# ruizhecao96/CMGAN

Hardware: NVIDIA H100
Metric: utterances/sec (2 s @16 kHz) generator fwd+bwd (higher is better)
Workload: dtype tf32

## Files before the change

### cmgan_b200/csrc/attention_mma.cu

```cuda
#include <type_traits>

#include "common.cuh"
#include "../../include/cmgan_b200.h"
#include "tc_ptx.cuh"

namespace {
using cmgan_tc::cp_async16;
using cmgan_tc::cp_async_commit;
using cmgan_tc::cp_async_wait;
using cmgan_tc::smem_u32;

constexpr int D = 16, H = 4, CQ = 64, LDQ = 192;
constexpr int QB = 64;
constexpr int KT = 64;
constexpr int LDS_ = 20;
constexpr int EW = QB + KT - 1;
constexpr int RW = 80;
constexpr int LDR = 84;
constexpr int MAXPOS = 512;
constexpr float SCALE_LOG2E = 0.25f * 1.4426950408889634f;

__device__ __forceinline__ float tf32r(float x) {
    uint32_t r;
    asm("cvt.rna.tf32.f32 %0, %1;" : "=r"(r) : "f"(x));
    return __uint_as_float(r);
}
__device__ __forceinline__ float tf32q(float x) { return __uint_as_float(__float_as_uint(x) + 0x1000u); }
__device__ __forceinline__ float ex2(float x) {
    float y;
    asm("ex2.approx.ftz.f32 %0, %1;" : "=f"(y) : "f"(x));
    return y;
}
__device__ __forceinline__ void mma_tf32(float c[4], const float a[4], float b0, float b1) {
    asm volatile("mma.sync.aligned.m16n8k8.row.col.f32.tf32.tf32.f32 {%0, %1, %2, %3}, {%4, %5, %6, %7}, {%8, %9}, {%0, %1, %2, %3};"
                 : "+f"(c[0]), "+f"(c[1]), "+f"(c[2]), "+f"(c[3])
                 : "r"(__float_as_uint(a[0])), "r"(__float_as_uint(a[1])), "r"(__float_as_uint(a[2])), "r"(__float_as_uint(a[3])),
                   "r"(__float_as_uint(b0)), "r"(__float_as_uint(b1)));
}
__device__ __forceinline__ int clampi(int v, int lo, int hi) { return v < lo ? lo : (v > hi ? hi : v); }

constexpr int EROWS = EW + 1;
constexpr int TILE_FLOATS = 2 * KT * LDS_ + EROWS * LDS_;
__device__ __forceinline__ void stage_tile_async(float* buf, const float* __restrict__ a_src, int a_ld, const float* __restrict__ b_src, int b_ld,
                                                 long base, long tok_stride, int first, int L, const float* __restrict__ E, int rfirst, int tid) {
    const uint32_t sa = smem_u32(buf), sb = sa + KT * LDS_ * 4, se = sb + KT * LDS_ * 4;
    for (int idx = tid; idx < KT * 4; idx += 128) {
        const int r = idx >> 2, q4 = idx & 3;
        const bool ok = first + r < L;
        const long row = base + (long)(ok ? first + r : 0) * tok_stride;
        cp_async16(sa + (r * LDS_ + q4 * 4) * 4, a_src + row * a_ld + q4 * 4, ok ? 16u : 0u);
        cp_async16(sb + (r * LDS_ + q4 * 4) * 4, b_src + row * b_ld + q4 * 4, ok ? 16u : 0u);
    }
    for (int idx = tid; idx < EROWS * 4; idx += 128) {
        const int w = idx >> 2, q4 = idx & 3;
        const int e = clampi(rfirst + w, -MAXPOS, MAXPOS) + MAXPOS;
        cp_async16(se + (w * LDS_ + q4 * 4) * 4, E + e * D + q4 * 4, 16u);
    }
}

template <int NBUF, bool RAGGED>
__global__ void __launch_bounds__(128) attn_fwd_mma_kernel(const float* __restrict__ qkv, SeqGeom g, const float* __restrict__ E,
                                                           float* __restrict__ ctx, float* __restrict__ lse, const int* __restrict__ tlen,
                                                           int axis) {
    extern __shared__ __align__(16) float smem_fwd[];
    float* Rs0 = smem_fwd + NBUF * TILE_FLOATS;
    const int s = blockIdx.x / H, h = blockIdx.x % H;
    const int i0 = blockIdx.y * QB;
    const int tid = threadIdx.x, warp = tid >> 5, lane = tid & 31, gq = lane >> 2, t = lane & 3;
    const int L = RAGGED ? ragged_seq_len(g, s, tlen, axis) : g.L;
    if (RAGGED && i0 >= L) return;
    const long base = seq_base(g, s);
    const int iw = i0 + warp * 16;
    const bool warp_active = iw < L;

    float qa[2][4];
#pragma unroll
    for (int ks = 0; ks < 2; ++ks)
#pragma unroll
        for (int r = 0; r < 4; ++r) {
            const int row = iw + gq + (r & 1) * 8, col = t + (r >> 1) * 4 + ks * 8;
            float v = 0.f;
            if (row < L) v = __ldg(qkv + (base + (long)row * g.tok_stride) * LDQ + h * D + col) * SCALE_LOG2E;
            qa[ks][r] = tf32r(v);
        }
    float o[2][4];
#pragma unroll
    for (int nd = 0; nd < 2; ++nd)
#pragma unroll
        for (int r = 0; r < 4; ++r) o[nd][r] = 0.f;
    float mrun[2] = {-INFINITY, -INFINITY}, lrun[2] = {0.f, 0.f};

    const float* ksrc = qkv + h * D + CQ;
    const float* vsrc = qkv + h * D + 2 * CQ;
    if (NBUF == 2) {
        stage_tile_async(smem_fwd, ksrc, LDQ, vsrc, LDQ, base, g.tok_stride, 0, L, E, i0 - (KT - 1), tid);
        cp_async_commit();
    }
    for (int j0 = 0, it = 0; j0 < L; j0 += KT, ++it) {
        const int nk = min(KT, L - j0);
        const float* Ks = smem_fwd + (NBUF == 2 ? (it & 1) : 0) * TILE_FLOATS;
        const float* Vs = Ks + KT * LDS_;
        const float* Es = Vs + KT * LDS_;
        __syncthreads();
        if (NBUF == 2) {
            if (j0 + KT < L)
                stage_tile_async(smem_fwd + ((it + 1) & 1) * TILE_FLOATS, ksrc, LDQ, vsrc, LDQ, base, g.tok_stride, j0 + KT, L, E,
                                 i0 - (j0 + KT) - (KT - 1), tid);
            cp_async_commit();
            cp_async_wait<1>();
        } else {
            stage_tile_async(smem_fwd, ksrc, LDQ, vsrc, LDQ, base, g.tok_stride, j0, L, E, i0 - j0 - (KT - 1), tid);
            cp_async_commit();
            cp_async_wait<0>();
        }
        __syncthreads();
        if (!warp_active) continue;
        auto tile_body = [&](auto full_tag) {
        constexpr bool FULL = decltype(full_tag)::value;
        const int ntv = (nk + 7) >> 3;
        const int rt0 = (KT - nk) >> 3;

        float sc[8][4];
#pragma unroll
        for (int nt = 0; nt < 8; ++nt) {
            sc[nt][0] = sc[nt][1] = sc[nt][2] = sc[nt][3] = 0.f;
            if (!FULL && nt >= ntv) continue;
#pragma unroll
            for (int ks = 0; ks < 2; ++ks) {
                const float* kp = Ks + (nt * 8 + gq) * LDS_ + t + ks * 8;
                mma_tf32(sc[nt], qa[ks], kp[0], kp[4]);
            }
        }
        float* R = Rs0 + warp * 16 * LDR;
#pragma unroll
        for (int nt = 0; nt < RW / 8; ++nt) {
            if (!FULL && nt < rt0) continue;
            float rc[4] = {0.f, 0.f, 0.f, 0.f};
#pragma unroll
            for (int ks = 0; ks < 2; ++ks) {
                const float* ep = Es + (warp * 16 + nt * 8 + gq) * LDS_ + t + ks * 8;
                mma_tf32(rc, qa[ks], ep[0], ep[4]);
            }
            *reinterpret_cast<float2*>(R + gq * LDR + nt * 8 + 2 * t) = make_float2(rc[0], rc[1]);
            *reinterpret_cast<float2*>(R + (gq + 8) * LDR + nt * 8 + 2 * t) = make_float2(rc[2], rc[3]);
        }
        __syncwarp();
        float tmax[2] = {-INFINITY, -INFINITY};
#pragma unroll
        for (int nt = 0; nt < 8; ++nt) {
            if (!FULL && nt >= ntv) { sc[nt][0] = sc[nt][1] = sc[nt][2] = sc[nt][3] = -INFINITY; continue; }
#pragma unroll
            for (int r = 0; r < 4; ++r) {
                const int qrow = gq + (r >> 1) * 8, kcol = nt * 8 + 2 * t + (r & 1);
                float v = sc[nt][r] + R[qrow * LDR + qrow - kcol + (KT - 1)];
                if (!FULL && kcol >= nk) v = -INFINITY;
                sc[nt][r] = v;
                tmax[r >> 1] = fmaxf(tmax[r >> 1], v);
            }
        }
        __syncwarp();
        float corr[2];
#pragma unroll
        for (int hrow = 0; hrow < 2; ++hrow) {
            float m = tmax[hrow];
            m = fmaxf(m, __shfl_xor_sync(0xffffffffu, m, 1));
            m = fmaxf(m, __shfl_xor_sync(0xffffffffu, m, 2));
            const float mnew = fmaxf(mrun[hrow], m);
            corr[hrow] = ex2(mrun[hrow] - mnew);
            mrun[hrow] = mnew;
            lrun[hrow] *= corr[hrow];
        }
#pragma unroll
        for (int nd = 0; nd < 2; ++nd) { o[nd][0] *= corr[0]; o[nd][1] *= corr[0]; o[nd][2] *= corr[1]; o[nd][3] *= corr[1]; }
#pragma unroll
        for (int nt = 0; nt < 8; ++nt) {
            if (!FULL && nt >= ntv) continue;
#pragma unroll
            for (int r = 0; r < 4; ++r) {
                const float p = ex2(sc[nt][r] - mrun[r >> 1]);
                lrun[r >> 1] += p;
                sc[nt][r] = tf32q(p);
            }
        }
#pragma unroll
        for (int kk = 0; kk < 8; ++kk) {
            if (!FULL && kk >= ntv) continue;
            const float pa[4] = {sc[kk][0], sc[kk][2], sc[kk][1], sc[kk][3]};
#pragma unroll
            for (int nd = 0; nd < 2; ++nd) {
                const float* vp = Vs + (kk * 8 + 2 * t) * LDS_ + nd * 8 + gq;
                mma_tf32(o[nd], pa, vp[0], vp[LDS_]);
            }
        }
        };
        if (nk == KT) tile_body(std::true_type{}); else tile_body(std::false_type{});
    }
    if (!warp_active) return;
#pragma unroll
    for (int hrow = 0; hrow < 2; ++hrow) {
        float l = lrun[hrow];
        l += __shfl_xor_sync(0xffffffffu, l, 1);
        l += __shfl_xor_sync(0xffffffffu, l, 2);
        lrun[hrow] = l;
    }
#pragma unroll
    for (int hrow = 0; hrow < 2; ++hrow) {
        const int i = iw + gq + hrow * 8;
        if (i >= L) continue;
        const float inv = 1.f / lrun[hrow];
        const long row = base + (long)i * g.tok_stride;
#pragma unroll
        for (int nd = 0; nd < 2; ++nd)
            *reinterpret_cast<float2*>(ctx + row * CQ + h * D + nd * 8 + 2 * t) = make_float2(tf32r(o[nd][hrow * 2] * inv), tf32r(o[nd][hrow * 2 + 1] * inv));
        if (lse && t == 0) lse[row * H + h] = mrun[hrow] + log2f(lrun[hrow]);
    }
}


constexpr float LN2 = 0.6931471805599453f;

__global__ void attn_delta_kernel(const float* __restrict__ ctx, const float* __restrict__ dctx, long n, float* __restrict__ delta) {
    const long i = (long)blockIdx.x * blockDim.x + threadIdx.x;
    if (i >= n) return;
    const float4* o = reinterpret_cast<const float4*>(ctx + i * D);
    const float4* d = reinterpret_cast<const float4*>(dctx + i * D);
    float acc = 0.f;
#pragma unroll
    for (int k = 0; k < 4; ++k) {
        const float4 a = __ldg(o + k), b = __ldg(d + k);
        acc = fmaf(a.x, b.x, acc); acc = fmaf(a.y, b.y, acc); acc = fmaf(a.z, b.z, acc); acc = fmaf(a.w, b.w, acc);
    }
    delta[i] = acc;
}

constexpr int LDRB = 136;
template <bool GDE>
__global__ void __launch_bounds__(128, GDE ? 3 : 2) attn_bwd_dq_mma_kernel(const float* __restrict__ qkv, SeqGeom g, const float* __restrict__ E,
                                                              const float* __restrict__ ctx, const float* __restrict__ dctx,
                                                              const float* __restrict__ lse, int n_items, int Lpad,
                                                              float* __restrict__ delta, float* __restrict__ dqkv,
                                                              float* __restrict__ dE, float* __restrict__ de_scratch) {
    extern __shared__ __align__(16) float smem_dq[];
    constexpr int NBUF = GDE ? 1 : 2;
    float* Rb = smem_dq + NBUF * TILE_FLOATS;
    float* Qs = Rb + QB * LDRB;
    float* dEs = GDE ? de_scratch + ((long)blockIdx.y * gridDim.x + blockIdx.x) * (long)(Lpad + 64) * D : Qs + QB * LDS_;
    const int i0 = blockIdx.y * QB;
    const int tid = threadIdx.x, warp = tid >> 5, lane = tid & 31, gq = lane >> 2, t = lane & 3;
    const int iw = i0 + warp * 16;
    const bool warp_active = iw < g.L;
    const int acc_rows = Lpad + 64;
    const int r_acc0 = i0 - Lpad + 1;
    for (int idx = tid; idx < acc_rows * D; idx += 128) dEs[idx] = 0.f;
    for (int idx = tid; idx < QB * LDRB; idx += 128) Rb[idx] = 0.f;
    float* R = Rb + warp * 16 * LDRB + warp * 16;
    float* Qw = Qs + warp * 16 * LDS_;

    auto stage = [&](int item, int j0, int slot) {
        const int s = item / H, h = item % H;
        stage_tile_async(smem_dq + slot * TILE_FLOATS, qkv + h * D + CQ, LDQ, qkv + h * D + 2 * CQ, LDQ, seq_base(g, s), g.tok_stride, j0, g.L, E,
                         i0 - j0 - (KT - 1), tid);
    };
    if (!GDE) {
        if ((int)blockIdx.x < n_items) stage(blockIdx.x, 0, 0);
        cp_async_commit();
    }
    int it = 0;
    float qn[2][4], dn[2][4], dln[2], lsn[2];
    auto fetch_item = [&](int item) {
        const int s = item / H, h = item % H;
        const long base = seq_base(g, s);
#pragma unroll
        for (int ks = 0; ks < 2; ++ks)
#pragma unroll
            for (int r = 0; r < 4; ++r) {
                const int row = iw + gq + (r & 1) * 8, col = t + (r >> 1) * 4 + ks * 8;
                float qv = 0.f, dv = 0.f;
                if (row < g.L) {
                    const long rr = base + (long)row * g.tok_stride;
                    qv = __ldg(qkv + rr * LDQ + h * D + col);
                    dv = __ldg(dctx + rr * CQ + h * D + col);
                }
                qn[ks][r] = qv;
                dn[ks][r] = dv;
            }
#pragma unroll
        for (int hrow = 0; hrow < 2; ++hrow) {
            const int row = iw + gq + hrow * 8;
            lsn[hrow] = 0.f; dln[hrow] = 0.f;
            if (row < g.L) {
                const long rr = base + (long)row * g.tok_stride;
                lsn[hrow] = __ldg(lse + rr * H + h);
                dln[hrow] = __ldg(delta + rr * H + h);
            }
        }
    };
    if (!GDE && (int)blockIdx.x < n_items) fetch_item(blockIdx.x);
    for (int item = blockIdx.x; item < n_items; item += gridDim.x) {
        const int s = item / H, h = item % H;
        const long base = seq_base(g, s);
        if (GDE) fetch_item(item);
        float qa[2][4], da[2][4], dl[2], ls[2];
#pragma unroll
        for (int ks = 0; ks < 2; ++ks)
#pragma unroll
            for (int r = 0; r < 4; ++r) {
                qa[ks][r] = tf32r(qn[ks][r] * SCALE_LOG2E);
                da[ks][r] = tf32r(dn[ks][r]);
            }
        dl[0] = dln[0]; dl[1] = dln[1]; ls[0] = lsn[0]; ls[1] = lsn[1];
        float dq[2][4];
#pragma unroll
        for (int nd = 0; nd < 2; ++nd)
#pragma unroll
            for (int r = 0; r < 4; ++r) dq[nd][r] = 0.f;

        for (int j0 = 0; j0 < g.L; j0 += KT) {
            const int nk = min(KT, g.L - j0);
            __syncthreads();
            if (j0 == 0) {
#pragma unroll
                for (int ks = 0; ks < 2; ++ks)
#pragma unroll
                    for (int r = 0; r < 4; ++r) Qw[(gq + (r & 1) * 8) * LDS_ + t + (r >> 1) * 4 + ks * 8] = qa[ks][r];
            }
            if (GDE) {
                stage(item, j0, 0);
                cp_async_commit();
                cp_async_wait<0>();
            } else {
                if (j0 + KT < g.L) stage(item, j0 + KT, (it + 1) & 1);
                else if (item + (int)gridDim.x < n_items) {
                    stage(item + gridDim.x, 0, (it + 1) & 1);
                    fetch_item(item + gridDim.x);
                }
                cp_async_commit();
                cp_async_wait<1>();
            }
            __syncthreads();
            const float* Ks = smem_dq + (GDE ? 0 : (it & 1)) * TILE_FLOATS;
            const float* Vs = Ks + KT * LDS_;
            const float* Es = Vs + KT * LDS_;
            ++it;
            auto tile_body = [&](auto full_tag) {
            constexpr bool FULL = decltype(full_tag)::value;
            const int ntv = (nk + 7) >> 3;
            const int rt0 = (KT - nk) >> 3;
            if (warp_active) {
                float sc[8][4], dp[8][4];
#pragma unroll
                for (int nt = 0; nt < 8; ++nt) {
                    sc[nt][0] = sc[nt][1] = sc[nt][2] = sc[nt][3] = 0.f;
                    dp[nt][0] = dp[nt][1] = dp[nt][2] = dp[nt][3] = 0.f;
                    if (!FULL && nt >= ntv) continue;
#pragma unroll
                    for (int ks = 0; ks < 2; ++ks) {
                        const float* kp = Ks + (nt * 8 + gq) * LDS_ + t + ks * 8;
                        const float* vp = Vs + (nt * 8 + gq) * LDS_ + t + ks * 8;
                        mma_tf32(sc[nt], qa[ks], kp[0], kp[4]);
                        mma_tf32(dp[nt], da[ks], vp[0], vp[4]);
                    }
                }
#pragma unroll
                for (int nt = 0; nt < RW / 8; ++nt) {
                    if (!FULL && nt < rt0) continue;
                    float rc[4] = {0.f, 0.f, 0.f, 0.f};
#pragma unroll
                    for (int ks = 0; ks < 2; ++ks) {
                        const float* ep = Es + (warp * 16 + nt * 8 + gq) * LDS_ + t + ks * 8;
                        mma_tf32(rc, qa[ks], ep[0], ep[4]);
                    }
                    *reinterpret_cast<float2*>(R + gq * LDRB + nt * 8 + 2 * t) = make_float2(rc[0], rc[1]);
                    *reinterpret_cast<float2*>(R + (gq + 8) * LDRB + nt * 8 + 2 * t) = make_float2(rc[2], rc[3]);
                }
                __syncwarp();
#pragma unroll
                for (int nt = 0; nt < 8; ++nt) {
                    if (!FULL && nt >= ntv) continue;
#pragma unroll
                    for (int r = 0; r < 4; ++r) {
                        const int qrow = gq + (r >> 1) * 8, kcol = nt * 8 + 2 * t + (r & 1);
                        const float a = sc[nt][r] + R[qrow * LDRB + qrow - kcol + (KT - 1)];
                        float ds = ex2(a - ls[r >> 1]) * (dp[nt][r] - dl[r >> 1]);
                        if (!FULL && kcol >= nk) ds = 0.f;
                        sc[nt][r] = tf32q(ds);
                    }
                }
                __syncwarp();
#pragma unroll
                for (int u = 0; u < 8; ++u) {
                    const int idx = lane + 32 * u, row = idx >> 4, c = (row + 64 + (idx & 15)) % RW;
                    R[row * LDRB + c] = 0.f;
                }
#pragma unroll
                for (int nt = 0; nt < 8; ++nt)
#pragma unroll
                    for (int r = 0; r < 4; ++r) {
                        const int qrow = gq + (r >> 1) * 8, kcol = nt * 8 + 2 * t + (r & 1);
                        R[qrow * LDRB + qrow - kcol + (KT - 1)] = sc[nt][r];
                    }
                __syncwarp();
#pragma unroll
                for (int kk = 0; kk < 8; ++kk) {
                    if (!FULL && kk >= ntv) continue;
                    const float pa[4] = {sc[kk][0], sc[kk][2], sc[kk][1], sc[kk][3]};
#pragma unroll
                    for (int nd = 0; nd < 2; ++nd) {
                        const float* kp = Ks + (kk * 8 + 2 * t) * LDS_ + nd * 8 + gq;
                        mma_tf32(dq[nd], pa, kp[0], kp[LDS_]);
                    }
                }
#pragma unroll
                for (int kk = 0; kk < RW / 8; ++kk) {
                    if (!FULL && kk < rt0) continue;
                    const float ra[4] = {R[gq * LDRB + kk * 8 + t], R[(gq + 8) * LDRB + kk * 8 + t], R[gq * LDRB + kk * 8 + t + 4],
                                         R[(gq + 8) * LDRB + kk * 8 + t + 4]};
#pragma unroll
                    for (int nd = 0; nd < 2; ++nd) {
                        const float* ep = Es + (warp * 16 + kk * 8 + t) * LDS_ + nd * 8 + gq;
                        mma_tf32(dq[nd], ra, ep[0], ep[4 * LDS_]);
                    }
                }
            }
            __syncthreads();
            {
                const int arow0 = (i0 - j0 - (KT - 1)) - r_acc0 + warp * 32;
#pragma unroll
                for (int mt = 0; mt < 2; ++mt) {
                    if (!FULL && warp * 32 + mt * 16 + 16 <= KT - nk) continue;
                    float ec[2][4] = {{0.f, 0.f, 0.f, 0.f}, {0.f, 0.f, 0.f, 0.f}};
#pragma unroll
                    for (int ks = 0; ks < QB / 8; ++ks) {
                        const float* rp = Rb + (t + 8 * ks) * LDRB + warp * 32 + 16 * mt + gq;
                        const float ta[4] = {rp[0], rp[8], rp[4 * LDRB], rp[4 * LDRB + 8]};
#pragma unroll
                        for (int nd = 0; nd < 2; ++nd) {
                            const float* qp = Qs + (t + 8 * ks) * LDS_ + nd * 8 + gq;
                            mma_tf32(ec[nd], ta, qp[0], qp[4 * LDS_]);
                        }
                    }
#pragma unroll
                    for (int nd = 0; nd < 2; ++nd)
#pragma unroll
                        for (int hrow = 0; hrow < 2; ++hrow) {
                            float2* ap = reinterpret_cast<float2*>(dEs + (arow0 + 16 * mt + gq + hrow * 8) * D + nd * 8 + 2 * t);
                            float2 v = *ap;
                            v.x += ec[nd][hrow * 2]; v.y += ec[nd][hrow * 2 + 1];
                            *ap = v;
                        }
                }
            }
            };
            if (nk == KT) tile_body(std::true_type{}); else tile_body(std::false_type{});
        }
        if (warp_active) {
#pragma unroll
            for (int hrow = 0; hrow < 2; ++hrow) {
                const int i = iw + gq + hrow * 8;
                if (i >= g.L) continue;
                const long row = base + (long)i * g.tok_stride;
#pragma unroll
                for (int nd = 0; nd < 2; ++nd)
                    *reinterpret_cast<float2*>(dqkv + row * LDQ + h * D + nd * 8 + 2 * t) =
                        make_float2(tf32r(0.25f * dq[nd][hrow * 2]), tf32r(0.25f * dq[nd][hrow * 2 + 1]));
            }
        }
    }
    __syncthreads();
    for (int idx = tid; idx < acc_rows * D; idx += 128) {
        const int rr = r_acc0 + idx / D;
        if (rr < -(g.L - 1) || rr > g.L - 1) continue;
        const float v = dEs[idx];
        if (v != 0.f) atomicAdd(dE + (clampi(rr, -MAXPOS, MAXPOS) + MAXPOS) * D + (idx % D), v * LN2);
    }
}

constexpr int LDR2 = 132;
__global__ void __launch_bounds__(128, 3) attn_bwd_dkv_mma_kernel(const float* __restrict__ qkv, SeqGeom g, const float* __restrict__ E,
                                                               const float* __restrict__ dctx, const float* __restrict__ lse,
                                                               const float* __restrict__ delta, float* __restrict__ dqkv) {
    extern __shared__ __align__(16) float smem_kv[];
    float* R2 = smem_kv + 2 * TILE_FLOATS;
    float* LD = R2 + QB * LDR2;
    const int s = blockIdx.x / H, h = blockIdx.x % H;
    const int j0 = blockIdx.y * KT;
    const int tid = threadIdx.x, warp = tid >> 5, lane = tid & 31, gq = lane >> 2, t = lane & 3;
    const long base = seq_base(g, s);
    const int jw = j0 + warp * 16;
    const bool warp_active = jw < g.L;

    float ka[2][4], va[2][4];
#pragma unroll
    for (int ks = 0; ks < 2; ++ks)
#pragma unroll
        for (int r = 0; r < 4; ++r) {
            const int row = jw + gq + (r & 1) * 8, col = t + (r >> 1) * 4 + ks * 8;
            float kv = 0.f, vv = 0.f;
            if (row < g.L) {
                const float* p = qkv + (base + (long)row * g.tok_stride) * LDQ + h * D + col;
                kv = __ldg(p + CQ);
                vv = __ldg(p + 2 * CQ);
            }
            ka[ks][r] = tf32r(kv * SCALE_LOG2E);
            va[ks][r] = tf32r(vv);
        }
    float dk[2][4], dv[2][4];
#pragma unroll
    for (int nd = 0; nd < 2; ++nd)
#pragma unroll
        for (int r = 0; r < 4; ++r) { dk[nd][r] = 0.f; dv[nd][r] = 0.f; }
    for (int idx = tid; idx < QB * LDR2; idx += 128) R2[idx] = 0.f;

    const float* qsrc = qkv + h * D;
    const float* osrc = dctx + h * D;
    auto stage = [&](int i0, int slot) {
        stage_tile_async(smem_kv + slot * TILE_FLOATS, qsrc, LDQ, osrc, CQ, base, g.tok_stride, i0, g.L, E, i0 - j0 - (KT - 1), tid);
        const int r = tid & 63;
        const bool ok = i0 + r < g.L;
        const long rr = base + (long)(ok ? i0 + r : 0) * g.tok_stride;
        const float* src = (tid < 64 ? lse : delta) + rr * H + h;
        asm volatile("cp.async.ca.shared.global [%0], [%1], 4, %2;" ::"r"(smem_u32(LD + slot * 2 * QB + tid)), "l"(src), "r"(ok ? 4u : 0u) : "memory");
    };
    stage(0, 0);
    cp_async_commit();
    for (int i0 = 0, it = 0; i0 < g.L; i0 += QB, ++it) {
        const int nq = min(QB, g.L - i0);
        __syncthreads();
        if (i0 + QB < g.L) stage(i0 + QB, (it + 1) & 1);
        cp_async_commit();
        cp_async_wait<1>();
        __syncthreads();
        const float* Qs = smem_kv + (it & 1) * TILE_FLOATS;
        const float* Os = Qs + QB * LDS_;
        const float* Es = Os + QB * LDS_;
        const float* Ls = LD + (it & 1) * 2 * QB;
        const float* Dl = Ls + QB;
        auto tile_body = [&](auto full_tag) {
        constexpr bool FULL = decltype(full_tag)::value;
        {
            float qa[2][4];
#pragma unroll
            for (int ks = 0; ks < 2; ++ks)
#pragma unroll
                for (int r = 0; r < 4; ++r) qa[ks][r] = Qs[(warp * 16 + gq + (r & 1) * 8) * LDS_ + t + (r >> 1) * 4 + ks * 8] * SCALE_LOG2E;
            const int ntr = FULL ? 16 : (warp * 16 < nq ? min(16, ((nq + 62) >> 3) + 1) : 0);
#pragma unroll 4
            for (int nt = 0; nt < ntr; ++nt) {
                float rc[4] = {0.f, 0.f, 0.f, 0.f};
#pragma unroll
                for (int ks = 0; ks < 2; ++ks) {
                    const float* ep = Es + (nt * 8 + gq) * LDS_ + t + ks * 8;
                    mma_tf32(rc, qa[ks], ep[0], ep[4]);
                }
                *reinterpret_cast<float2*>(R2 + (warp * 16 + gq) * LDR2 + nt * 8 + 2 * t) = make_float2(rc[0], rc[1]);
                *reinterpret_cast<float2*>(R2 + (warp * 16 + gq + 8) * LDR2 + nt * 8 + 2 * t) = make_float2(rc[2], rc[3]);
            }
        }
        __syncthreads();
        if (!warp_active) return;
        const int ntq = (nq + 7) >> 3;

        float sc[8][4], dp[8][4];
#pragma unroll
        for (int nt = 0; nt < 8; ++nt) {
            sc[nt][0] = sc[nt][1] = sc[nt][2] = sc[nt][3] = 0.f;
            dp[nt][0] = dp[nt][1] = dp[nt][2] = dp[nt][3] = 0.f;
            if (!FULL && nt >= ntq) continue;
#pragma unroll
            for (int ks = 0; ks < 2; ++ks) {
                const float* qp = Qs + (nt * 8 + gq) * LDS_ + t + ks * 8;
                const float* op = Os + (nt * 8 + gq) * LDS_ + t + ks * 8;
                mma_tf32(sc[nt], ka[ks], qp[0], qp[4]);
                mma_tf32(dp[nt], va[ks], op[0], op[4]);
            }
        }
#pragma unroll
        for (int nt = 0; nt < 8; ++nt) {
            if (!FULL && nt >= ntq) continue;
            const float2 l2 = *reinterpret_cast<const float2*>(Ls + nt * 8 + 2 * t);
            const float2 d2 = *reinterpret_cast<const float2*>(Dl + nt * 8 + 2 * t);
#pragma unroll
            for (int r = 0; r < 4; ++r) {
                const int jl = warp * 16 + gq + (r >> 1) * 8, il = nt * 8 + 2 * t + (r & 1);
                const float a = sc[nt][r] + R2[il * LDR2 + il - jl + (KT - 1)];
                float p = ex2(a - ((r & 1) ? l2.y : l2.x));
                if (!FULL && il >= nq) p = 0.f;
                sc[nt][r] = tf32q(p);
                dp[nt][r] = tf32q(p * (dp[nt][r] - ((r & 1) ? d2.y : d2.x)));
            }
        }
#pragma unroll
        for (int kk = 0; kk < 8; ++kk) {
            if (!FULL && kk >= ntq) continue;
            const float pa[4] = {sc[kk][0], sc[kk][2], sc[kk][1], sc[kk][3]};
            const float sa[4] = {dp[kk][0], dp[kk][2], dp[kk][1], dp[kk][3]};
#pragma unroll
            for (int nd = 0; nd < 2; ++nd) {
                const float* op = Os + (kk * 8 + 2 * t) * LDS_ + nd * 8 + gq;
                const float* qp = Qs + (kk * 8 + 2 * t) * LDS_ + nd * 8 + gq;
                mma_tf32(dv[nd], pa, op[0], op[LDS_]);
                mma_tf32(dk[nd], sa, qp[0], qp[LDS_]);
            }
        }
        };
        if (nq == QB) tile_body(std::true_type{}); else tile_body(std::false_type{});
    }
    if (!warp_active) return;
#pragma unroll
    for (int hrow = 0; hrow < 2; ++hrow) {
        const int j = jw + gq + hrow * 8;
        if (j >= g.L) continue;
        float* p = dqkv + (base + (long)j * g.tok_stride) * LDQ + h * D + 2 * t;
#pragma unroll
        for (int nd = 0; nd < 2; ++nd) {
            *reinterpret_cast<float2*>(p + CQ + nd * 8) = make_float2(tf32r(0.25f * dk[nd][hrow * 2]), tf32r(0.25f * dk[nd][hrow * 2 + 1]));
            *reinterpret_cast<float2*>(p + 2 * CQ + nd * 8) = make_float2(tf32r(dv[nd][hrow * 2]), tf32r(dv[nd][hrow * 2 + 1]));
        }
    }
}

}

constexpr int FWD_NBUF_DEFAULT = 1;
CMGAN_API int cmgan_attention_fwd_tf32(const float* qkv, const float* E, int B, int T, int F, int axis, float* ctx, float* lse, void* stream) {
    return cmgan_attention_fwd_tf32_nbuf(qkv, E, B, T, F, axis, ctx, lse, FWD_NBUF_DEFAULT, stream);
}

static int attention_fwd_tf32_launch(const float* qkv, const float* E, int B, int T, int F, int axis, const int* tlen, float* ctx, float* lse,
                                     int nbuf, void* stream) {
    CMGAN_REQUIRE(qkv && E && ctx, "cmgan_attention_fwd_tf32: null pointer");
    CMGAN_REQUIRE(nbuf == 1 || nbuf == 2, "cmgan_attention_fwd_tf32_nbuf: nbuf must be 1 or 2");
    CMGAN_REQUIRE(axis == 0 || axis == 1, "cmgan_attention_fwd_tf32: axis must be 0 (time) or 1 (freq)");
    SeqGeom g = make_seq_geom(B, T, F, axis);
    if (g.n_seq == 0 || g.L == 0) return 0;
    dim3 grid(g.n_seq * H, cdiv(g.L, QB));
    const int smem = (nbuf * TILE_FLOATS + 4 * 16 * LDR) * (int)sizeof(float);
    static bool attr_set = false;
    if (!attr_set) {
        const int smem2 = (2 * TILE_FLOATS + 4 * 16 * LDR) * (int)sizeof(float);
        cudaError_t e = cudaFuncSetAttribute(attn_fwd_mma_kernel<2, false>, cudaFuncAttributeMaxDynamicSharedMemorySize, smem2);
        if (e == cudaSuccess) e = cudaFuncSetAttribute(attn_fwd_mma_kernel<2, true>, cudaFuncAttributeMaxDynamicSharedMemorySize, smem2);
        CMGAN_REQUIRE(e == cudaSuccess, "cmgan_attention_fwd_tf32: cudaFuncSetAttribute: %s", cudaGetErrorString(e));
        attr_set = true;
    }
    cudaStream_t st = (cudaStream_t)stream;
    if (tlen) {
        if (nbuf == 2) attn_fwd_mma_kernel<2, true><<<grid, 128, smem, st>>>(qkv, g, E, ctx, lse, tlen, axis);
        else attn_fwd_mma_kernel<1, true><<<grid, 128, smem, st>>>(qkv, g, E, ctx, lse, tlen, axis);
    } else {
        if (nbuf == 2) attn_fwd_mma_kernel<2, false><<<grid, 128, smem, st>>>(qkv, g, E, ctx, lse, nullptr, axis);
        else attn_fwd_mma_kernel<1, false><<<grid, 128, smem, st>>>(qkv, g, E, ctx, lse, nullptr, axis);
    }
    return cmgan_check_launch("attn_fwd_mma_kernel");
}

CMGAN_API int cmgan_attention_fwd_tf32_nbuf(const float* qkv, const float* E, int B, int T, int F, int axis, float* ctx, float* lse, int nbuf,
                                            void* stream) {
    return attention_fwd_tf32_launch(qkv, E, B, T, F, axis, nullptr, ctx, lse, nbuf, stream);
}

CMGAN_API int cmgan_attention_fwd_tf32_ragged(const float* qkv, const float* E, int B, int T, int F, int axis, const int* frames, float* ctx,
                                              float* lse, void* stream) {
    CMGAN_REQUIRE(frames, "cmgan_attention_fwd_tf32_ragged: frames is null");
    return attention_fwd_tf32_launch(qkv, E, B, T, F, axis, frames, ctx, lse, FWD_NBUF_DEFAULT, stream);
}

static int dq_blocks(int ntile, int per_sm, int n_items) {
    int ng = (cmgan_num_sms() * per_sm) / ntile;
    if (ng < 1) ng = 1;
    return ng > n_items ? n_items : ng;
}

CMGAN_API long long cmgan_attention_bwd_ws_floats(int B, int T, int F, int axis) {
    if (axis != 0 && axis != 1) { cmgan_set_error("cmgan_attention_bwd_ws_floats: axis must be 0 (time) or 1 (freq)"); return -1; }
    SeqGeom g = make_seq_geom(B, T, F, axis);
    if (g.n_seq == 0 || g.L == 0) return 0;
    const int ntile = cdiv(g.L, QB), Lpad = ntile * KT;
    return (long long)dq_blocks(ntile, 3, g.n_seq * H) * ntile * (Lpad + 64) * D;
}

CMGAN_API int cmgan_attention_bwd_tf32_ws(const float* qkv, const float* E, const float* ctx, const float* dctx, const float* lse, int B,
                                          int T, int F, int axis, float* delta, float* dqkv, float* dE, int parts, float* scratch,
                                          long long scratch_floats, void* stream) {
    CMGAN_REQUIRE(qkv && E && ctx && dctx && lse && delta && dqkv && dE, "cmgan_attention_bwd_tf32: null pointer");
    CMGAN_REQUIRE(axis == 0 || axis == 1, "cmgan_attention_bwd_tf32: axis must be 0 (time) or 1 (freq)");
    SeqGeom g = make_seq_geom(B, T, F, axis);
    if (g.n_seq == 0 || g.L == 0) return 0;
    cudaStream_t st = (cudaStream_t)stream;
    const int ntile = cdiv(g.L, QB), Lpad = ntile * KT;
    const int n_items = g.n_seq * H;
    const bool gde = scratch != nullptr;
    if (gde) CMGAN_REQUIRE(scratch_floats >= cmgan_attention_bwd_ws_floats(B, T, F, axis) && (((uintptr_t)scratch) & 7) == 0,
                           "cmgan_attention_bwd_tf32_ws: scratch too small (%lld floats) or misaligned", scratch_floats);
    const int smem_dq = ((gde ? 1 : 2) * TILE_FLOATS + QB * LDRB + QB * LDS_ + (gde ? 0 : (Lpad + 64) * D)) * (int)sizeof(float);
    const int smem_kv = (2 * TILE_FLOATS + QB * LDR2 + 4 * QB) * (int)sizeof(float);
    CMGAN_REQUIRE(smem_dq <= 227 * 1024, "cmgan_attention_bwd_tf32: sequence length %d too long for the shared dE accumulator", g.L);
    static int smem_dq_set = 0;
    static bool kv_set = false, gde_set = false;
    if (!gde && smem_dq > smem_dq_set) {
        cudaError_t e = cudaFuncSetAttribute(attn_bwd_dq_mma_kernel<false>, cudaFuncAttributeMaxDynamicSharedMemorySize, smem_dq);
        CMGAN_REQUIRE(e == cudaSuccess, "cmgan_attention_bwd_tf32: cudaFuncSetAttribute: %s", cudaGetErrorString(e));
        smem_dq_set = smem_dq;
    }
    if (gde && !gde_set) {
        cudaError_t e = cudaFuncSetAttribute(attn_bwd_dq_mma_kernel<true>, cudaFuncAttributeMaxDynamicSharedMemorySize, smem_dq);
        CMGAN_REQUIRE(e == cudaSuccess, "cmgan_attention_bwd_tf32: cudaFuncSetAttribute: %s", cudaGetErrorString(e));
        gde_set = true;
    }
    if (!kv_set) {
        cudaError_t e = cudaFuncSetAttribute(attn_bwd_dkv_mma_kernel, cudaFuncAttributeMaxDynamicSharedMemorySize, smem_kv);
        CMGAN_REQUIRE(e == cudaSuccess, "cmgan_attention_bwd_tf32: cudaFuncSetAttribute: %s", cudaGetErrorString(e));
        kv_set = true;
    }
    if (parts & 1) {
        const long n = (long)B * T * F * H;
        attn_delta_kernel<<<cdiv(n, 256), 256, 0, st>>>(ctx, dctx, n, delta);
        if (cmgan_check_launch("attn_delta_kernel")) return -1;
    }
    if (parts & 2) {
        if (gde)
            attn_bwd_dq_mma_kernel<true><<<dim3(dq_blocks(ntile, 3, n_items), ntile), 128, smem_dq, st>>>(qkv, g, E, ctx, dctx, lse, n_items, Lpad,
                                                                                                          delta, dqkv, dE, scratch);
        else
            attn_bwd_dq_mma_kernel<false><<<dim3(dq_blocks(ntile, 2, n_items), ntile), 128, smem_dq, st>>>(qkv, g, E, ctx, dctx, lse, n_items, Lpad,
                                                                                                           delta, dqkv, dE, nullptr);
        if (cmgan_check_launch("attn_bwd_dq_mma_kernel")) return -1;
    }
    if (parts & 4) {
        attn_bwd_dkv_mma_kernel<<<dim3(n_items, ntile), 128, smem_kv, st>>>(qkv, g, E, dctx, lse, delta, dqkv);
        if (cmgan_check_launch("attn_bwd_dkv_mma_kernel")) return -1;
    }
    return 0;
}

CMGAN_API int cmgan_attention_bwd_tf32_parts(const float* qkv, const float* E, const float* ctx, const float* dctx, const float* lse, int B,
                                             int T, int F, int axis, float* delta, float* dqkv, float* dE, int parts, void* stream) {
    return cmgan_attention_bwd_tf32_ws(qkv, E, ctx, dctx, lse, B, T, F, axis, delta, dqkv, dE, parts, nullptr, 0, stream);
}

CMGAN_API int cmgan_attention_bwd_tf32(const float* qkv, const float* E, const float* ctx, const float* dctx, const float* lse, int B,
                                       int T, int F, int axis, float* delta, float* dqkv, float* dE, void* stream) {
    return cmgan_attention_bwd_tf32_parts(qkv, E, ctx, dctx, lse, B, T, F, axis, delta, dqkv, dE, 7, stream);
}
```

### cmgan_b200/csrc/tc_ptx.cuh

```cuda
#pragma once
#include "common.cuh"

namespace cmgan_tc {

__device__ __forceinline__ uint32_t smem_u32(const void* p) { return (uint32_t)__cvta_generic_to_shared(p); }

__device__ __forceinline__ void mbar_init(uint32_t bar, uint32_t count) {
    asm volatile("mbarrier.init.shared::cta.b64 [%0], %1;" ::"r"(bar), "r"(count) : "memory");
}
__device__ __forceinline__ void mbar_arrive(uint32_t bar) {
    asm volatile("mbarrier.arrive.shared::cta.b64 _, [%0];" ::"r"(bar) : "memory");
}
__device__ __forceinline__ void mbar_arrive_expect_tx(uint32_t bar, uint32_t bytes) {
    asm volatile("mbarrier.arrive.expect_tx.shared::cta.b64 _, [%0], %1;" ::"r"(bar), "r"(bytes) : "memory");
}
__device__ __forceinline__ void mbar_wait(uint32_t bar, uint32_t parity) {
    uint32_t done = 0;
    for (uint32_t spin = 0; !done; ++spin) {
        asm volatile("{\n\t.reg .pred p;\n\tmbarrier.try_wait.parity.shared::cta.b64 p, [%1], %2;\n\tselp.u32 %0, 1, 0, p;\n\t}"
                     : "=r"(done) : "r"(bar), "r"(parity) : "memory");
        if (spin > (1u << 28)) __trap();
    }
}
__device__ __forceinline__ bool mbar_test(uint32_t bar, uint32_t parity) {
    uint32_t done;
    asm volatile("{\n\t.reg .pred p;\n\tmbarrier.test_wait.parity.shared::cta.b64 p, [%1], %2;\n\tselp.u32 %0, 1, 0, p;\n\t}"
                 : "=r"(done) : "r"(bar), "r"(parity) : "memory");
    return done != 0;
}
__device__ __forceinline__ void fence_barrier_init() { asm volatile("fence.mbarrier_init.release.cluster;" ::: "memory"); }
__device__ __forceinline__ void fence_proxy_async() { asm volatile("fence.proxy.async.shared::cta;" ::: "memory"); }

__device__ __forceinline__ void bulk_g2s(uint32_t dst_smem, const void* src, uint32_t bytes, uint32_t bar) {
    asm volatile("cp.async.bulk.shared::cluster.global.mbarrier::complete_tx::bytes [%0], [%1], %2, [%3];"
                 ::"r"(dst_smem), "l"(src), "r"(bytes), "r"(bar) : "memory");
}
__device__ __forceinline__ void tma_load_2d(uint32_t dst_smem, const void* tmap, int c0, int c1, uint32_t bar) {
    asm volatile("cp.async.bulk.tensor.2d.shared::cluster.global.mbarrier::complete_tx::bytes [%0], [%1, {%2, %3}], [%4];"
                 ::"r"(dst_smem), "l"(tmap), "r"(c0), "r"(c1), "r"(bar) : "memory");
}
__device__ __forceinline__ void tma_load_3d(uint32_t dst_smem, const void* tmap, int c0, int c1, int c2, uint32_t bar) {
    asm volatile("cp.async.bulk.tensor.3d.shared::cluster.global.mbarrier::complete_tx::bytes [%0], [%1, {%2, %3, %4}], [%5];"
                 ::"r"(dst_smem), "l"(tmap), "r"(c0), "r"(c1), "r"(c2), "r"(bar) : "memory");
}
__device__ __forceinline__ void tma_load_4d(uint32_t dst_smem, const void* tmap, int c0, int c1, int c2, int c3, uint32_t bar) {
    asm volatile("cp.async.bulk.tensor.4d.shared::cluster.global.mbarrier::complete_tx::bytes [%0], [%1, {%2, %3, %4, %5}], [%6];"
                 ::"r"(dst_smem), "l"(tmap), "r"(c0), "r"(c1), "r"(c2), "r"(c3), "r"(bar) : "memory");
}
__device__ __forceinline__ void cp_async16(uint32_t dst_smem, const void* src, uint32_t src_bytes) {
    asm volatile("cp.async.cg.shared.global [%0], [%1], 16, %2;" ::"r"(dst_smem), "l"(src), "r"(src_bytes) : "memory");
}
__device__ __forceinline__ void cp_async8(uint32_t dst_smem, const void* src) {
    asm volatile("cp.async.ca.shared.global [%0], [%1], 8;" ::"r"(dst_smem), "l"(src) : "memory");
}
__device__ __forceinline__ void cp_async_commit() { asm volatile("cp.async.commit_group;" ::: "memory"); }
template <int N>
__device__ __forceinline__ void cp_async_wait() { asm volatile("cp.async.wait_group %0;" ::"n"(N) : "memory"); }

__device__ __forceinline__ float to_tf32(float x) {
    uint32_t r;
    asm("cvt.rna.tf32.f32 %0, %1;" : "=r"(r) : "f"(x));
    return __uint_as_float(r);
}

__device__ __forceinline__ uint64_t gmma_desc_sw128(uint32_t saddr) {
    uint64_t d = 0;
    d |= (uint64_t)((saddr & 0x3FFFF) >> 4);
    d |= (uint64_t)1 << 16;
    d |= (uint64_t)(1024 >> 4) << 32;
    d |= (uint64_t)1 << 62;
    return d;
}
__device__ __forceinline__ void wgmma_fence() { asm volatile("wgmma.fence.sync.aligned;" ::: "memory"); }
__device__ __forceinline__ void wgmma_commit() { asm volatile("wgmma.commit_group.sync.aligned;" ::: "memory"); }
template <int N>
__device__ __forceinline__ void wgmma_wait() { asm volatile("wgmma.wait_group.sync.aligned %0;" ::"n"(N) : "memory"); }
__device__ __forceinline__ void wgmma_m64n16k8_tf32(float d[8], uint64_t adesc, uint64_t bdesc, uint32_t accumulate) {
    asm volatile("{\n\t.reg .pred p;\n\tsetp.ne.b32 p, %10, 0;\n\t"
                 "wgmma.mma_async.sync.aligned.m64n16k8.f32.tf32.tf32 {%0, %1, %2, %3, %4, %5, %6, %7}, %8, %9, p, 1, 1;\n\t}"
                 : "+f"(d[0]), "+f"(d[1]), "+f"(d[2]), "+f"(d[3]), "+f"(d[4]), "+f"(d[5]), "+f"(d[6]), "+f"(d[7])
                 : "l"(adesc), "l"(bdesc), "r"(accumulate));
}
#define CMGAN_D8(b) "+f"(d[b][0]), "+f"(d[b][1]), "+f"(d[b][2]), "+f"(d[b][3]), "+f"(d[b][4]), "+f"(d[b][5]), "+f"(d[b][6]), "+f"(d[b][7])
__device__ __forceinline__ void wgmma_m64n64k8_tf32(float (&d)[4][8], uint64_t adesc, uint64_t bdesc, uint32_t accumulate) {
    asm volatile("{\n\t.reg .pred p;\n\tsetp.ne.b32 p, %34, 0;\n\t"
                 "wgmma.mma_async.sync.aligned.m64n64k8.f32.tf32.tf32 "
                 "{%0, %1, %2, %3, %4, %5, %6, %7, %8, %9, %10, %11, %12, %13, %14, %15, "
                 "%16, %17, %18, %19, %20, %21, %22, %23, %24, %25, %26, %27, %28, %29, %30, %31}, %32, %33, p, 1, 1;\n\t}"
                 : CMGAN_D8(0), CMGAN_D8(1), CMGAN_D8(2), CMGAN_D8(3)
                 : "l"(adesc), "l"(bdesc), "r"(accumulate));
}
__device__ __forceinline__ void wgmma_m64n64k8_tf32_rs(float (&d)[4][8], const uint32_t (&a)[4], uint64_t bdesc, uint32_t accumulate) {
    asm volatile("{\n\t.reg .pred p;\n\tsetp.ne.b32 p, %37, 0;\n\t"
                 "wgmma.mma_async.sync.aligned.m64n64k8.f32.tf32.tf32 "
                 "{%0, %1, %2, %3, %4, %5, %6, %7, %8, %9, %10, %11, %12, %13, %14, %15, "
                 "%16, %17, %18, %19, %20, %21, %22, %23, %24, %25, %26, %27, %28, %29, %30, %31}, {%32, %33, %34, %35}, %36, p, 1, 1;\n\t}"
                 : CMGAN_D8(0), CMGAN_D8(1), CMGAN_D8(2), CMGAN_D8(3)
                 : "r"(a[0]), "r"(a[1]), "r"(a[2]), "r"(a[3]), "l"(bdesc), "r"(accumulate));
}
#undef CMGAN_D8

template <int NB, int NBMAX>
__device__ __forceinline__ void mma_chunk(float (&acc)[NBMAX][8], uint64_t adesc, uint64_t bdesc, bool first) {
#pragma unroll
    for (int k = 0; k < 4; ++k)
#pragma unroll
        for (int j = 0; j < NB; ++j)
            wgmma_m64n16k8_tf32(acc[j], adesc + (uint64_t)(2 * k), bdesc + (uint64_t)(128 * j + 2 * k), (first && k == 0) ? 0u : 1u);
}
template <int NBMAX, int I = 1>
__device__ __forceinline__ void mma_chunk_n(int nb, float (&acc)[NBMAX][8], uint64_t adesc, uint64_t bdesc, bool first) {
    if constexpr (I <= NBMAX) {
        if (nb == I) mma_chunk<I, NBMAX>(acc, adesc, bdesc, first);
        else mma_chunk_n<NBMAX, I + 1>(nb, acc, adesc, bdesc, first);
    }
}

}
```

Before: 84.26.

## Use warpgroup wgmma with swizzled smem tiles for attention backward logits

Moves the QK, dO·V and relative-position logit products in the dq and dkv attention backward kernels from per-warp mma.sync to warpgroup wgmma. A-fragments come from registers, and K/V/E tiles are staged into a new 64B-swizzled shared-memory layout. The cp.async pipeline now waits fully and adds a proxy fence each step, and the dq kernel hoists Q fragments out of its dE loop. This trades finer per-warp masking and some copy/compute overlap for larger asynchronous tensor-core instructions. It also raises the shared-memory alignment requirement.

```diff
diff --git a/cmgan_b200/csrc/attention_mma.cu b/cmgan_b200/csrc/attention_mma.cu
--- a/cmgan_b200/csrc/attention_mma.cu
+++ b/cmgan_b200/csrc/attention_mma.cu
@@ -219,6 +219,45 @@
 
 constexpr float LN2 = 0.6931471805599453f;
 
+using cmgan_tc::gmma_desc_sw64;
+using cmgan_tc::wgmma_commit;
+using cmgan_tc::wgmma_fence;
+using cmgan_tc::wgmma_m64n64k8_tf32_rs;
+using cmgan_tc::wgmma_wait;
+constexpr int GROWS = KT * D;
+constexpr int BTILE_FLOATS = 2 * GROWS + EROWS * D;
+__device__ __forceinline__ int bidx(int r, int k) { return r * D + ((((k >> 2) ^ (r >> 1)) & 3) << 2) + (k & 3); }
+__device__ __forceinline__ uint64_t bdesc(const float* tile, int row0, int ks) {
+    return gmma_desc_sw64(smem_u32(tile) + row0 * D * 4 + ks * 32);
+}
+__device__ __forceinline__ void stage_tile_bwd(float* buf, const float* __restrict__ a_src, int a_ld, const float* __restrict__ b_src, int b_ld,
+                                               long base, long tok_stride, int first, int L, const float* __restrict__ E, int rfirst, int tid) {
+    const uint32_t sa = smem_u32(buf), sb = sa + GROWS * 4, se = sb + GROWS * 4;
+    for (int idx = tid; idx < KT * 4; idx += 128) {
+        const int r = idx >> 2, q4 = idx & 3;
+        const bool ok = first + r < L;
+        const long row = base + (long)(ok ? first + r : 0) * tok_stride;
+        cp_async16(sa + bidx(r, q4 * 4) * 4, a_src + row * a_ld + q4 * 4, ok ? 16u : 0u);
+        cp_async16(sb + bidx(r, q4 * 4) * 4, b_src + row * b_ld + q4 * 4, ok ? 16u : 0u);
+    }
+    for (int idx = tid; idx < EROWS * 4; idx += 128) {
+        const int w = idx >> 2, q4 = idx & 3;
+        const int e = clampi(rfirst + w, -MAXPOS, MAXPOS) + MAXPOS;
+        cp_async16(se + bidx(w, q4 * 4) * 4, E + e * D + q4 * 4, 16u);
+    }
+}
+__device__ __forceinline__ void wg_logits(float (&acc)[8][4], const uint32_t (&a)[2][4], const float* tile, int row0) {
+    float (&d)[4][8] = reinterpret_cast<float (&)[4][8]>(acc);
+    wgmma_m64n64k8_tf32_rs(d, a[0], bdesc(tile, row0, 0), 0u);
+    wgmma_m64n64k8_tf32_rs(d, a[1], bdesc(tile, row0, 1), 1u);
+}
+__device__ __forceinline__ void to_bits(uint32_t (&u)[2][4], const float (&f)[2][4]) {
+#pragma unroll
+    for (int ks = 0; ks < 2; ++ks)
+#pragma unroll
+        for (int r = 0; r < 4; ++r) u[ks][r] = __float_as_uint(f[ks][r]);
+}
+
 __global__ void attn_delta_kernel(const float* __restrict__ ctx, const float* __restrict__ dctx, long n, float* __restrict__ delta) {
     const long i = (long)blockIdx.x * blockDim.x + threadIdx.x;
     if (i >= n) return;
@@ -240,9 +279,9 @@
                                                               const float* __restrict__ lse, int n_items, int Lpad,
                                                               float* __restrict__ delta, float* __restrict__ dqkv,
                                                               float* __restrict__ dE, float* __restrict__ de_scratch) {
-    extern __shared__ __align__(16) float smem_dq[];
+    extern __shared__ __align__(1024) float smem_dq[];
     constexpr int NBUF = GDE ? 1 : 2;
-    float* Rb = smem_dq + NBUF * TILE_FLOATS;
+    float* Rb = smem_dq + NBUF * BTILE_FLOATS;
     float* Qs = Rb + QB * LDRB;
     float* dEs = GDE ? de_scratch + ((long)blockIdx.y * gridDim.x + blockIdx.x) * (long)(Lpad + 64) * D : Qs + QB * LDS_;
     const int i0 = blockIdx.y * QB;
@@ -258,7 +297,7 @@
 
     auto stage = [&](int item, int j0, int slot) {
         const int s = item / H, h = item % H;
-        stage_tile_async(smem_dq + slot * TILE_FLOATS, qkv + h * D + CQ, LDQ, qkv + h * D + 2 * CQ, LDQ, seq_base(g, s), g.tok_stride, j0, g.L, E,
+        stage_tile_bwd(smem_dq + slot * BTILE_FLOATS, qkv + h * D + CQ, LDQ, qkv + h * D + 2 * CQ, LDQ, seq_base(g, s), g.tok_stride, j0, g.L, E,
                          i0 - j0 - (KT - 1), tid);
     };
     if (!GDE) {
@@ -308,6 +347,9 @@
                 qa[ks][r] = tf32r(qn[ks][r] * SCALE_LOG2E);
                 da[ks][r] = tf32r(dn[ks][r]);
             }
+        uint32_t qu[2][4], du[2][4];
+        to_bits(qu, qa);
+        to_bits(du, da);
         dl[0] = dln[0]; dl[1] = dln[1]; ls[0] = lsn[0]; ls[1] = lsn[1];
         float dq[2][4];
 #pragma unroll
@@ -327,52 +369,52 @@
             if (GDE) {
                 stage(item, j0, 0);
                 cp_async_commit();
-                cp_async_wait<0>();
-            } else {
+            }
+            cp_async_wait<0>();
+            cmgan_tc::fence_proxy_async();
+            __syncthreads();
+            if (!GDE) {
                 if (j0 + KT < g.L) stage(item, j0 + KT, (it + 1) & 1);
                 else if (item + (int)gridDim.x < n_items) {
                     stage(item + gridDim.x, 0, (it + 1) & 1);
                     fetch_item(item + gridDim.x);
                 }
                 cp_async_commit();
-                cp_async_wait<1>();
-            }
-            __syncthreads();
-            const float* Ks = smem_dq + (GDE ? 0 : (it & 1)) * TILE_FLOATS;
-            const float* Vs = Ks + KT * LDS_;
-            const float* Es = Vs + KT * LDS_;
+            }
+            const float* Ks = smem_dq + (GDE ? 0 : (it & 1)) * BTILE_FLOATS;
+            const float* Vs = Ks + GROWS;
+            const float* Es = Vs + GROWS;
             ++it;
             auto tile_body = [&](auto full_tag) {
             constexpr bool FULL = decltype(full_tag)::value;
             const int ntv = (nk + 7) >> 3;
             const int rt0 = (KT - nk) >> 3;
+            float sc[8][4], dp[8][4], rr[8][4];
+            wgmma_fence();
+            wg_logits(sc, qu, Ks, 0);
+            wg_logits(dp, du, Vs, 0);
+            wg_logits(rr, qu, Es, 0);
+            wgmma_commit();
+#pragma unroll
+            for (int half = 0; half < 2; ++half) {
+                wgmma_wait<0>();
+                if (warp_active) {
+#pragma unroll
+                    for (int nt = 0; nt < 8; ++nt) {
+                        const int c = half * 64 + nt * 8;
+                        if (c < 16 * warp || c >= 16 * warp + RW) continue;
+                        const float* rc = rr[nt];
+                        *reinterpret_cast<float2*>(Rb + (warp * 16 + gq) * LDRB + c + 2 * t) = make_float2(rc[0], rc[1]);
+                        *reinterpret_cast<float2*>(Rb + (warp * 16 + gq + 8) * LDRB + c + 2 * t) = make_float2(rc[2], rc[3]);
+                    }
+                }
+                if (half == 0) {
+                    wgmma_fence();
+                    wg_logits(rr, qu, Es, 64);
+                    wgmma_commit();
+                }
+            }
             if (warp_active) {
-                float sc[8][4], dp[8][4];
-#pragma unroll
-                for (int nt = 0; nt < 8; ++nt) {
-                    sc[nt][0] = sc[nt][1] = sc[nt][2] = sc[nt][3] = 0.f;
-                    dp[nt][0] = dp[nt][1] = dp[nt][2] = dp[nt][3] = 0.f;
-                    if (!FULL && nt >= ntv) continue;
-#pragma unroll
-                    for (int ks = 0; ks < 2; ++ks) {
-                        const float* kp = Ks + (nt * 8 + gq) * LDS_ + t + ks * 8;
-                        const float* vp = Vs + (nt * 8 + gq) * LDS_ + t + ks * 8;
-                        mma_tf32(sc[nt], qa[ks], kp[0], kp[4]);
-                        mma_tf32(dp[nt], da[ks], vp[0], vp[4]);
-                    }
-                }
-#pragma unroll
-                for (int nt = 0; nt < RW / 8; ++nt) {
-                    if (!FULL && nt < rt0) continue;
-                    float rc[4] = {0.f, 0.f, 0.f, 0.f};
-#pragma unroll
-                    for (int ks = 0; ks < 2; ++ks) {
-                        const float* ep = Es + (warp * 16 + nt * 8 + gq) * LDS_ + t + ks * 8;
-                        mma_tf32(rc, qa[ks], ep[0], ep[4]);
-                    }
-                    *reinterpret_cast<float2*>(R + gq * LDRB + nt * 8 + 2 * t) = make_float2(rc[0], rc[1]);
-                    *reinterpret_cast<float2*>(R + (gq + 8) * LDRB + nt * 8 + 2 * t) = make_float2(rc[2], rc[3]);
-                }
                 __syncwarp();
 #pragma unroll
                 for (int nt = 0; nt < 8; ++nt) {
@@ -406,8 +448,8 @@
                     const float pa[4] = {sc[kk][0], sc[kk][2], sc[kk][1], sc[kk][3]};
 #pragma unroll
                     for (int nd = 0; nd < 2; ++nd) {
-                        const float* kp = Ks + (kk * 8 + 2 * t) * LDS_ + nd * 8 + gq;
-                        mma_tf32(dq[nd], pa, kp[0], kp[LDS_]);
+                        const float* kp = Ks + bidx(kk * 8 + 2 * t, nd * 8 + gq);
+                        mma_tf32(dq[nd], pa, kp[0], kp[D]);
                     }
                 }
 #pragma unroll
@@ -417,14 +459,23 @@
                                          R[(gq + 8) * LDRB + kk * 8 + t + 4]};
 #pragma unroll
                     for (int nd = 0; nd < 2; ++nd) {
-                        const float* ep = Es + (warp * 16 + kk * 8 + t) * LDS_ + nd * 8 + gq;
-                        mma_tf32(dq[nd], ra, ep[0], ep[4 * LDS_]);
+                        const int er = warp * 16 + kk * 8 + t;
+                        mma_tf32(dq[nd], ra, Es[bidx(er, nd * 8 + gq)], Es[bidx(er + 4, nd * 8 + gq)]);
                     }
                 }
             }
             __syncthreads();
             {
                 const int arow0 = (i0 - j0 - (KT - 1)) - r_acc0 + warp * 32;
+                float qb[QB / 8][2][2];
+#pragma unroll
+                for (int ks = 0; ks < QB / 8; ++ks)
+#pragma unroll
+                    for (int nd = 0; nd < 2; ++nd) {
+                        const float* qp = Qs + (t + 8 * ks) * LDS_ + nd * 8 + gq;
+                        qb[ks][nd][0] = qp[0];
+                        qb[ks][nd][1] = qp[4 * LDS_];
+                    }
 #pragma unroll
                 for (int mt = 0; mt < 2; ++mt) {
                     if (!FULL && warp * 32 + mt * 16 + 16 <= KT - nk) continue;
@@ -434,10 +485,7 @@
                         const float* rp = Rb + (t + 8 * ks) * LDRB + warp * 32 + 16 * mt + gq;
                         const float ta[4] = {rp[0], rp[8], rp[4 * LDRB], rp[4 * LDRB + 8]};
 #pragma unroll
-                        for (int nd = 0; nd < 2; ++nd) {
-                            const float* qp = Qs + (t + 8 * ks) * LDS_ + nd * 8 + gq;
-                            mma_tf32(ec[nd], ta, qp[0], qp[4 * LDS_]);
-                        }
+                        for (int nd = 0; nd < 2; ++nd) mma_tf32(ec[nd], ta, qb[ks][nd][0], qb[ks][nd][1]);
                     }
 #pragma unroll
                     for (int nd = 0; nd < 2; ++nd)
@@ -479,8 +527,8 @@
 __global__ void __launch_bounds__(128, 3) attn_bwd_dkv_mma_kernel(const float* __restrict__ qkv, SeqGeom g, const float* __restrict__ E,
                                                                const float* __restrict__ dctx, const float* __restrict__ lse,
                                                                const float* __restrict__ delta, float* __restrict__ dqkv) {
-    extern __shared__ __align__(16) float smem_kv[];
-    float* R2 = smem_kv + 2 * TILE_FLOATS;
+    extern __shared__ __align__(1024) float smem_kv[];
+    float* R2 = smem_kv + 2 * BTILE_FLOATS;
     float* LD = R2 + QB * LDR2;
     const int s = blockIdx.x / H, h = blockIdx.x % H;
     const int j0 = blockIdx.y * KT;
@@ -489,7 +537,7 @@
     const int jw = j0 + warp * 16;
     const bool warp_active = jw < g.L;
 
-    float ka[2][4], va[2][4];
+    uint32_t ka[2][4], va[2][4];
 #pragma unroll
     for (int ks = 0; ks < 2; ++ks)
 #pragma unroll
@@ -501,20 +549,19 @@
                 kv = __ldg(p + CQ);
                 vv = __ldg(p + 2 * CQ);
             }
-            ka[ks][r] = tf32r(kv * SCALE_LOG2E);
-            va[ks][r] = tf32r(vv);
+            ka[ks][r] = __float_as_uint(tf32r(kv * SCALE_LOG2E));
+            va[ks][r] = __float_as_uint(tf32r(vv));
         }
     float dk[2][4], dv[2][4];
 #pragma unroll
     for (int nd = 0; nd < 2; ++nd)
 #pragma unroll
         for (int r = 0; r < 4; ++r) { dk[nd][r] = 0.f; dv[nd][r] = 0.f; }
-    for (int idx = tid; idx < QB * LDR2; idx += 128) R2[idx] = 0.f;
 
     const float* qsrc = qkv + h * D;
     const float* osrc = dctx + h * D;
     auto stage = [&](int i0, int slot) {
-        stage_tile_async(smem_kv + slot * TILE_FLOATS, qsrc, LDQ, osrc, CQ, base, g.tok_stride, i0, g.L, E, i0 - j0 - (KT - 1), tid);
+        stage_tile_bwd(smem_kv + slot * BTILE_FLOATS, qsrc, LDQ, osrc, CQ, base, g.tok_stride, i0, g.L, E, i0 - j0 - (KT - 1), tid);
         const int r = tid & 63;
         const bool ok = i0 + r < g.L;
         const long rr = base + (long)(ok ? i0 + r : 0) * g.tok_stride;
@@ -525,55 +572,49 @@
     cp_async_commit();
     for (int i0 = 0, it = 0; i0 < g.L; i0 += QB, ++it) {
         const int nq = min(QB, g.L - i0);
+        cp_async_wait<0>();
+        cmgan_tc::fence_proxy_async();
         __syncthreads();
         if (i0 + QB < g.L) stage(i0 + QB, (it + 1) & 1);
         cp_async_commit();
-        cp_async_wait<1>();
-        __syncthreads();
-        const float* Qs = smem_kv + (it & 1) * TILE_FLOATS;
-        const float* Os = Qs + QB * LDS_;
-        const float* Es = Os + QB * LDS_;
+        const float* Qs = smem_kv + (it & 1) * BTILE_FLOATS;
+        const float* Os = Qs + GROWS;
+        const float* Es = Os + GROWS;
         const float* Ls = LD + (it & 1) * 2 * QB;
         const float* Dl = Ls + QB;
         auto tile_body = [&](auto full_tag) {
         constexpr bool FULL = decltype(full_tag)::value;
+        float sc[8][4], dp[8][4];
         {
             float qa[2][4];
 #pragma unroll
             for (int ks = 0; ks < 2; ++ks)
 #pragma unroll
-                for (int r = 0; r < 4; ++r) qa[ks][r] = Qs[(warp * 16 + gq + (r & 1) * 8) * LDS_ + t + (r >> 1) * 4 + ks * 8] * SCALE_LOG2E;
-            const int ntr = FULL ? 16 : (warp * 16 < nq ? min(16, ((nq + 62) >> 3) + 1) : 0);
-#pragma unroll 4
-            for (int nt = 0; nt < ntr; ++nt) {
-                float rc[4] = {0.f, 0.f, 0.f, 0.f};
-#pragma unroll
-                for (int ks = 0; ks < 2; ++ks) {
-                    const float* ep = Es + (nt * 8 + gq) * LDS_ + t + ks * 8;
-                    mma_tf32(rc, qa[ks], ep[0], ep[4]);
-                }
-                *reinterpret_cast<float2*>(R2 + (warp * 16 + gq) * LDR2 + nt * 8 + 2 * t) = make_float2(rc[0], rc[1]);
-                *reinterpret_cast<float2*>(R2 + (warp * 16 + gq + 8) * LDR2 + nt * 8 + 2 * t) = make_float2(rc[2], rc[3]);
-            }
-        }
+                for (int r = 0; r < 4; ++r) qa[ks][r] = Qs[bidx(warp * 16 + gq + (r & 1) * 8, t + (r >> 1) * 4 + ks * 8)] * SCALE_LOG2E;
+            uint32_t qu[2][4];
+            to_bits(qu, qa);
+            float rr[8][4];
+#pragma unroll
+            for (int half = 0; half < 2; ++half) {
+                wgmma_fence();
+                wg_logits(rr, qu, Es, half * 64);
+                wgmma_commit();
+                wgmma_wait<0>();
+#pragma unroll
+                for (int nt = 0; nt < 8; ++nt) {
+                    *reinterpret_cast<float2*>(R2 + (warp * 16 + gq) * LDR2 + half * 64 + nt * 8 + 2 * t) = make_float2(rr[nt][0], rr[nt][1]);
+                    *reinterpret_cast<float2*>(R2 + (warp * 16 + gq + 8) * LDR2 + half * 64 + nt * 8 + 2 * t) = make_float2(rr[nt][2], rr[nt][3]);
+                }
+            }
+        }
+        wgmma_fence();
+        wg_logits(sc, ka, Qs, 0);
+        wg_logits(dp, va, Os, 0);
+        wgmma_commit();
+        wgmma_wait<0>();
         __syncthreads();
         if (!warp_active) return;
         const int ntq = (nq + 7) >> 3;
-
-        float sc[8][4], dp[8][4];
-#pragma unroll
-        for (int nt = 0; nt < 8; ++nt) {
-            sc[nt][0] = sc[nt][1] = sc[nt][2] = sc[nt][3] = 0.f;
-            dp[nt][0] = dp[nt][1] = dp[nt][2] = dp[nt][3] = 0.f;
-            if (!FULL && nt >= ntq) continue;
-#pragma unroll
-            for (int ks = 0; ks < 2; ++ks) {
-                const float* qp = Qs + (nt * 8 + gq) * LDS_ + t + ks * 8;
-                const float* op = Os + (nt * 8 + gq) * LDS_ + t + ks * 8;
-                mma_tf32(sc[nt], ka[ks], qp[0], qp[4]);
-                mma_tf32(dp[nt], va[ks], op[0], op[4]);
-            }
-        }
 #pragma unroll
         for (int nt = 0; nt < 8; ++nt) {
             if (!FULL && nt >= ntq) continue;
@@ -596,10 +637,10 @@
             const float sa[4] = {dp[kk][0], dp[kk][2], dp[kk][1], dp[kk][3]};
 #pragma unroll
             for (int nd = 0; nd < 2; ++nd) {
-                const float* op = Os + (kk * 8 + 2 * t) * LDS_ + nd * 8 + gq;
-                const float* qp = Qs + (kk * 8 + 2 * t) * LDS_ + nd * 8 + gq;
-                mma_tf32(dv[nd], pa, op[0], op[LDS_]);
-                mma_tf32(dk[nd], sa, qp[0], qp[LDS_]);
+                const float* op = Os + bidx(kk * 8 + 2 * t, nd * 8 + gq);
+                const float* qp = Qs + bidx(kk * 8 + 2 * t, nd * 8 + gq);
+                mma_tf32(dv[nd], pa, op[0], op[D]);
+                mma_tf32(dk[nd], sa, qp[0], qp[D]);
             }
         }
         };
@@ -692,8 +733,8 @@
     const bool gde = scratch != nullptr;
     if (gde) CMGAN_REQUIRE(scratch_floats >= cmgan_attention_bwd_ws_floats(B, T, F, axis) && (((uintptr_t)scratch) & 7) == 0,
                            "cmgan_attention_bwd_tf32_ws: scratch too small (%lld floats) or misaligned", scratch_floats);
-    const int smem_dq = ((gde ? 1 : 2) * TILE_FLOATS + QB * LDRB + QB * LDS_ + (gde ? 0 : (Lpad + 64) * D)) * (int)sizeof(float);
-    const int smem_kv = (2 * TILE_FLOATS + QB * LDR2 + 4 * QB) * (int)sizeof(float);
+    const int smem_dq = ((gde ? 1 : 2) * BTILE_FLOATS + QB * LDRB + QB * LDS_ + (gde ? 0 : (Lpad + 64) * D)) * (int)sizeof(float);
+    const int smem_kv = (2 * BTILE_FLOATS + QB * LDR2 + 4 * QB) * (int)sizeof(float);
     CMGAN_REQUIRE(smem_dq <= 227 * 1024, "cmgan_attention_bwd_tf32: sequence length %d too long for the shared dE accumulator", g.L);
     static int smem_dq_set = 0;
     static bool kv_set = false, gde_set = false;
diff --git a/cmgan_b200/csrc/tc_ptx.cuh b/cmgan_b200/csrc/tc_ptx.cuh
--- a/cmgan_b200/csrc/tc_ptx.cuh
+++ b/cmgan_b200/csrc/tc_ptx.cuh
@@ -71,6 +71,14 @@
     d |= (uint64_t)1 << 62;
     return d;
 }
+__device__ __forceinline__ uint64_t gmma_desc_sw64(uint32_t saddr) {
+    uint64_t d = 0;
+    d |= (uint64_t)((saddr & 0x3FFFF) >> 4);
+    d |= (uint64_t)1 << 16;
+    d |= (uint64_t)(512 >> 4) << 32;
+    d |= (uint64_t)2 << 62;
+    return d;
+}
 __device__ __forceinline__ void wgmma_fence() { asm volatile("wgmma.fence.sync.aligned;" ::: "memory"); }
 __device__ __forceinline__ void wgmma_commit() { asm volatile("wgmma.commit_group.sync.aligned;" ::: "memory"); }
 template <int N>
```

Result: faster. 85.61 (median of 6 runs) (+1.6%).
